# SokhengDin/DNN-MPPI-MPC

Measured on AMD Instinct MI355X. Metric: trajectory-steps/sec (KxT/iter_time), diff-drive K=4096 T=50, higher is better.
Workload: dtype f32; 1 GPU; BASELINE config 2: differential-drive analytic dynamics, K=4096 x T=50 per GPU, reference __main__ parameters, closed loop with the driver's plant on the device; K_per_gpu=4096, K_global=4096, T=50, waypoint_mode=sequential (reference-exact), noise=Philox4x32-10 in-kernel, waypoint_idx_at_end_of_timing=99, build_id=03c7b1dc90acac61, exchange=none (one GPU)

## Files before the change

dnn-mppi-mpc_amd/csrc/mppi_kernels.hip:

```cpp
#include <hip/hip_runtime.h>
#include <limits.h>
#include <math.h>

#include "mppi_device.h"

namespace mppi {

template <typename R> struct alignas(4 * sizeof(R)) VecT4 { R x, y, z, w; };

#ifdef MPPI_STAMPS
__device__ unsigned long long g_stamps[128];
#define STAMP(n)                                                                 \
    do {                                                                         \
        if (blockIdx.x == gridDim.x - 1 && threadIdx.x == 0) g_stamps[64 + (n)] = wall_clock64(); \
        if (blockIdx.x == 0 && threadIdx.x == 0) {                               \
            g_stamps[n] = wall_clock64();                                        \
            if ((n) < 8) g_stamps[40 + (n)] = clock64();  \
            if ((n) == 16 || (n) == 21) g_stamps[32 + (n)] = clock64();           \
        }                                                                        \
    } while (0)
#else
#define STAMP(n) \
    do {         \
    } while (0)
// ... 1342 lines not shown
    }
    eta = wv::reduce<wv::OpAdd>(eta);
    eta2 = wv::reduce<wv::OpAdd>(eta2);
    n_hit = wv::reduce<wv::OpAdd>(n_hit);
    if (lane == 0) { sh_red[4 + wid] = eta; sh_red[8 + wid] = eta2; sh_red[12 + wid] = n_hit; }
    __syncthreads();
    R *out = partials + (size_t)blockIdx.x * record_len(P.T, (int)sizeof(R));
    if (tid == 0) {
        R a = 0, b = 0, nh = 0;
        for (int w = 0; w < nw; ++w) { a += sh_red[4 + w]; b += sh_red[8 + w]; nh += sh_red[12 + w]; }
        out[0] = rho;
        out[1] = a;
        out[2] = b;
        *reinterpret_cast<VecT4<R> *>(P.heads + 4 * (size_t)blockIdx.x) = VecT4<R>{rho, a, b, nh};
    }

    const int n_chunk = (P.T + 63) >> 6;
    for (int ch = 0; ch < n_chunk; ++ch) {
        const int t = ch * 64 + lane;
        R a0 = 0, a1 = 0;
        if (t < P.T) {
            for (int i = wid; i < nk; i += nw) {
                float e0, e1;
                if (P.use_philox) {
                    px::sample(P.seed_lo, P.seed_hi, iter, (unsigned)(k0 + i + P.k_offset), t, P.chol, e0, e1, (unsigned)P.noise_stream);
                } else {
                    const float2 e = *reinterpret_cast<const float2 *>(eps_tensor(P, iter, 0) + ((size_t)(k0 + i) * P.T + t) * 2);
                    e0 = e.x;
                    e1 = e.y;
                }
                const R w = sh_e[i];
                a0 += w * (R)e0;
                a1 += w * (R)e1;
            }
        }
        sh_acc[wid * 128 + 2 * lane] = a0;
        sh_acc[wid * 128 + 2 * lane + 1] = a1;
        __syncthreads();
        if (tid < 128 && ch * 64 + (tid >> 1) < P.T) {
            R s = 0;
            for (int w = 0; w < nw; ++w) s += sh_acc[w * 128 + tid];
            out[4 + ch * 128 + tid] = s;
        }
        __syncthreads();
    }
}

template <typename R>
__global__ void k_weights(const R *__restrict__ S, int K, double beta, double rho, double eta, double *w) {
    const int k = blockIdx.x * blockDim.x + threadIdx.x;
    if (k < K) w[k] = exp(-beta * ((double)S[k] - rho)) / eta;
}

template <int NT> struct MergeShape {
    static constexpr int GROUPS = NT / 32, MAXJ = MERGE_MAX_RECORDS / GROUPS, WAVES = NT / 64;
};

template <typename A> struct alignas(16) VecT { A v[16 / sizeof(A)]; };

template <typename A, int NT = MERGE_THREADS> struct MergeLds {
    A *w, *u, *s, *red, *part;
    __device__ __forceinline__ MergeLds(char *smem, int T, int W) {
        w = reinterpret_cast<A *>(smem);
        u = w + ((2 * (T + W + 1) + 3) & ~3);
        s = u + ((2 * T + 3) & ~3);
        red = s + MERGE_MAX_WINDOWS * NT;
        part = red + 64;
    }
};

__device__ __forceinline__ float fast_exp(float x) { return __expf(x); }
__device__ __forceinline__ double fast_exp(double x) { return exp(x); }
__device__ __forceinline__ float fast_div(float a, float b) { return a * __builtin_amdgcn_rcpf(b); }
__device__ __forceinline__ double fast_div(double a, double b) { return a / b; }

template <typename A> __device__ __forceinline__ void filter_store(A *sh_w, int i, A v, int T, int H, bool pad_copy) {
    const int t = i >> 1, d = i & 1;
    const A pv = pad_copy ? v : A(0);
    sh_w[2 * (t + H) + d] = v;
    if (t < H) sh_w[2 * t + d] = pv;
    if (t >= T - H) sh_w[2 * (t + 2 * H) + d] = pv;
    if (t == T - 1) sh_w[2 * (T + 2 * H) + d] = pv;
}
template <typename A> __device__ __forceinline__ A filter_at(const A *sh_w, int t, int d, int T, int W, int f_filter) {
    const int H = W / 2;
    const A inv_w = fast_div(A(1), (A)W);
    if (f_filter == FILTER_NONE) return sh_w[2 * (t + H) + d];
    if (f_filter == FILTER_TORCH) {
        A sacc = 0;
        for (int q = 0; q < W; ++q) {
            const int m = t - H + q;
            if (m >= 0) sacc += sh_w[2 * m + d] * inv_w;
        }
        return sacc;
    }
    const A *tap = sh_w + 2 * t + d;
    A sacc = 0;
    if (W == 10) {
#pragma unroll
        for (int q = 0; q < 10; ++q) sacc += tap[2 * (9 - q)] * inv_w;
    } else {
        for (int q = 0; q < W; ++q) sacc += tap[2 * (W - 1 - q)] * inv_w;
    }
    if (f_filter == FILTER_DIFF) {
        const int n_conv = (W + 1) / 2;
        if (t == 0) sacc *= fast_div((A)W, (A)n_conv);
        else if (t < n_conv) sacc *= fast_div((A)W, (A)(t + n_conv));
        if (t == T - 1)
            for (int q = 1; q < n_conv; ++q) sacc *= fast_div((A)W, (A)(q + n_conv - (W % 2)));
    }
    return sacc;
}

template <typename A> struct BlockRed {
    static __device__ __forceinline__ A min1(A v, A *sh, int tid) {
        v = wv::reduce<wv::OpMin>(v);
        __syncthreads();
        if ((tid & 63) == 0) sh[tid >> 6] = v;
        __syncthreads();
        A r = sh[0];
#pragma unroll
        for (int w = 1; w < MERGE_THREADS / 64; ++w) r = fmin(r, sh[w]);
        return r;
    }
    static __device__ __forceinline__ void add2(A &a, A &b, A *sh, int tid) {
        a = wv::reduce<wv::OpAdd>(a);
        b = wv::reduce<wv::OpAdd>(b);
        __syncthreads();
        if ((tid & 63) == 0) { sh[tid >> 6] = a; sh[32 + (tid >> 6)] = b; }
        __syncthreads();
        a = 0;
        b = 0;
#pragma unroll
        for (int w = 0; w < MERGE_THREADS / 64; ++w) { a += sh[w]; b += sh[32 + w]; }
    }
};

template <typename A, int NT = MERGE_THREADS, int NWIN = 1> struct MergeRegs {
    VecT<A> w[NWIN][MergeShape<NT>::MAXJ];
    A hr[4 * NWIN], he[4 * NWIN], he2[4 * NWIN];
    A hc[4 * NWIN];
};

template <typename A, int NT, int NWIN>
__device__ __forceinline__ void merge_load_heads(const A *__restrict__ heads, MergeRegs<A, NT, NWIN> &m) {
    const int lane = threadIdx.x & 63;
#pragma unroll
    for (int i = 0; i < 4 * NWIN; ++i) {
        const int b = lane + 64 * i;
        const size_t r = (size_t)b;
        const VecT4<A> hd = *reinterpret_cast<const VecT4<A> *>(heads + 4 * r);
        m.hr[i] = hd.x;
        m.he[i] = hd.y;
        m.he2[i] = hd.z;
        m.hc[i] = hd.w;
    }
}

template <typename A, int NT, int NWIN>
__device__ __forceinline__ void merge_load_tile(const A *__restrict__ recs, int T, int vt, MergeRegs<A, NT, NWIN> &m) {
    constexpr int VW = 16 / sizeof(A), MAXJ = MergeShape<NT>::MAXJ;
    const int tid = threadIdx.x, vc = tid & 31, grp = tid >> 5;
    const unsigned rbytes = (unsigned)record_len(T, (int)sizeof(A)) * (unsigned)sizeof(A);
    const int nvc = (2 * T + VW - 1) / VW;
    const char *base = reinterpret_cast<const char *>(recs);
    const unsigned col = (unsigned)(4 + min(vt * 32 + vc, nvc - 1) * VW) * (unsigned)sizeof(A);
    const unsigned off0 = (unsigned)(grp * MAXJ) * rbytes + col;
#pragma unroll
    for (int win = 0; win < NWIN; ++win)
#pragma unroll
        for (int j = 0; j < MAXJ; ++j)
            m.w[win][j] = *reinterpret_cast<const VecT<A> *>(base + (off0 + (unsigned)(win * MERGE_MAX_RECORDS + j) * rbytes));
}

template <typename A, int NT, int NWIN, typename Store>
__device__ __forceinline__ void merge_combine(const A *__restrict__ recs, int n, int T, A beta,
                                              MergeRegs<A, NT, NWIN> &m, A *sh_s, A *sh_part, A &rho, A &eta, A &eta2,
                                              Store store, A *n_hit = nullptr) {
    constexpr int VW = 16 / sizeof(A), MAXJ = MergeShape<NT>::MAXJ, GROUPS = MergeShape<NT>::GROUPS;
    using V = VecT<A>;
    const int tid = threadIdx.x, lane = tid & 63, wid = tid >> 6;
    const int vc = tid & 31, grp = tid >> 5;
    const int nvc = (2 * T + VW - 1) / VW;
    A lr = A(INFINITY);
#pragma unroll
    for (int i = 0; i < 4 * NWIN; ++i) {
        if (lane + 64 * i >= n) m.hr[i] = A(INFINITY);
        lr = fmin(lr, m.hr[i]);
    }
    rho = wv::reduce<wv::OpMin>(lr);
    STAMP(25);
    A sc[4 * NWIN];
    eta = 0;
    eta2 = 0;
#pragma unroll
    for (int i = 0; i < 4 * NWIN; ++i) {
        sc[i] = lane + 64 * i < n ? fast_exp(-beta * (m.hr[i] - rho)) : A(0);
        eta += sc[i] * m.he[i];
        eta2 += sc[i] * sc[i] * m.he2[i];
    }
    eta = wv::reduce<wv::OpAdd>(eta);
    eta2 = wv::reduce<wv::OpAdd>(eta2);
    if (n_hit && *n_hit >= A(0)) {
        A cnt = 0;
#pragma unroll
        for (int i = 0; i < 4 * NWIN; ++i) cnt += lane + 64 * i < n ? m.hc[i] : A(0);
        *n_hit = wv::reduce<wv::OpAdd>(cnt);
    }
    const int r0 = wid * 2 * MAXJ, slot = r0 >> 6;
    A *my_s = sh_s + wid * 64;
#pragma unroll
    for (int win = 0; win < NWIN; ++win)
        my_s[win * NT + lane] = slot == 0 ? sc[4 * win] : slot == 1 ? sc[4 * win + 1] : slot == 2 ? sc[4 * win + 2] : sc[4 * win + 3];
    __builtin_amdgcn_fence(__ATOMIC_RELEASE, "wavefront");
    __builtin_amdgcn_wave_barrier();
    __builtin_amdgcn_fence(__ATOMIC_ACQUIRE, "wavefront");
    STAMP(26);
    const A *sj_base = my_s + (r0 & 63) + (grp & 1) * MAXJ;
    const A inv_eta = fast_div(A(1), eta);
    const int n_tiles = (nvc + 31) / 32;
    for (int vt = 0; vt < n_tiles; ++vt) {
        V acc;
#pragma unroll
        for (int q = 0; q < VW; ++q) acc.v[q] = 0;
#pragma unroll
        for (int win = 0; win < NWIN; ++win)
#pragma unroll
            for (int j = 0; j < MAXJ; ++j) {
                const A sj = sj_base[win * NT + j];
#pragma unroll
                for (int q = 0; q < VW; ++q) acc.v[q] += sj * m.w[win][j].v[q];
            }
        if (vt > 0) __syncthreads();
        *reinterpret_cast<V *>(sh_part + (grp * 32 + vc) * VW) = acc;
        __syncthreads();
        if (__builtin_expect(vt + 1 < n_tiles, 0)) merge_load_tile<A, NT, NWIN>(recs, T, vt + 1, m);
        for (int e = tid; e < 32 * VW; e += NT) {
            const int i = vt * 32 * VW + e;
            if (i < 2 * T) {
                A t = 0;
#pragma unroll
                for (int g = 0; g < GROUPS; ++g) t += sh_part[g * 32 * VW + e];
                store(i, t * inv_eta);
            }
        }
    }
    __syncthreads();
}

template <typename A, typename Store>
__device__ __forceinline__ void merge_abi(const double *recs, int n, int T, A beta, A *sh_s, A *sh_red, A &rho, A &eta,
                                          A &eta2, Store store, int stride = 0) {
    const int tid = threadIdx.x, plen = stride ? stride : partial_len(T);
    A hr = A(INFINITY), he = 0, he2 = 0;
    if (tid < n) {
        const double *pb = recs + tid * plen;
        hr = (A)pb[0];
        he = (A)pb[1];
        he2 = (A)pb[2];
    }
    rho = BlockRed<A>::min1(hr, sh_red, tid);
    const A sc = tid < n ? fast_exp(-beta * (hr - rho)) : A(0);
    if (tid < n) sh_s[tid] = sc;
    eta = sc * he;
    eta2 = sc * sc * he2;
    BlockRed<A>::add2(eta, eta2, sh_red, tid);
    const A inv_eta = fast_div(A(1), eta);
    for (int i = tid; i < 2 * T; i += MERGE_THREADS) {
        A t = 0;
        for (int b = 0; b < n; ++b) t += sh_s[b] * (A)recs[b * plen + 3 + i];
        store(i, t * inv_eta);
    }
    __syncthreads();
}

template <typename A, bool ABI_OUT>
__global__ __launch_bounds__(MERGE_THREADS) void k_merge(const A *__restrict__ recs, const A *__restrict__ heads, int n,
                                                         int group, int T, A beta, void *__restrict__ out,
                                                         A *__restrict__ out_heads) {
    extern __shared__ __attribute__((aligned(16))) char smem[];
    const MergeLds<A> L(smem, T, 0);
    A *sh_w = L.w;
    const int b0 = blockIdx.x * group, nb = min(group, n - b0);
    const A *mine = recs + (size_t)b0 * record_len(T, (int)sizeof(A));
    MergeRegs<A, MERGE_THREADS, 1> mr;
    merge_load_heads<A, MERGE_THREADS, 1>(heads + 4 * (size_t)b0, mr);
    merge_load_tile<A, MERGE_THREADS, 1>(mine, T, 0, mr);
    A rho, eta, eta2, n_hit = 0;
    merge_combine<A, MERGE_THREADS, 1>(mine, nb, T, beta, mr, L.s, L.part, rho, eta, eta2, [&](int i, A v) { sh_w[i] = v; }, &n_hit);
// ... 12 lines not shown
}

__device__ __forceinline__ char *peer_base(unsigned long long peer_ptr, int p) {
    const unsigned lo = (unsigned)__builtin_amdgcn_readlane((int)(unsigned)peer_ptr, p);
    const unsigned hi = (unsigned)__builtin_amdgcn_readlane((int)(unsigned)(peer_ptr >> 32), p);
    return reinterpret_cast<char *>(((unsigned long long)hi << 32) | lo);
}
__device__ __forceinline__ unsigned long long load_peer_ptrs(const FinalizeParams &F) {
    const int lane = threadIdx.x & 63;
    return lane < F.x_nranks ? reinterpret_cast<unsigned long long>(F.x_peers[lane]) : 0ull;
}

__device__ __forceinline__ bool exchange_flags(const FinalizeParams &F, unsigned long long peer_ptr, size_t slot_off) {
    const int tid = threadIdx.x;
    char *own = peer_base(peer_ptr, F.x_rank);
    __syncthreads();
    if (tid < F.x_nranks) {
        long long *theirs = reinterpret_cast<long long *>(reinterpret_cast<char *>(peer_ptr) + slot_off) + F.x_rank;
        __hip_atomic_store(theirs, F.x_seq, __ATOMIC_RELEASE, __HIP_MEMORY_SCOPE_SYSTEM);
        const long long *mine = reinterpret_cast<const long long *>(own + slot_off) + tid;
        const unsigned long long t0 = wall_clock64();
        while (__hip_atomic_load(mine, __ATOMIC_RELAXED, __HIP_MEMORY_SCOPE_SYSTEM) != F.x_seq) {
            if (wall_clock64() - t0 > (unsigned long long)F.x_timeout) {
                __hip_atomic_store(F.x_err, 1, __ATOMIC_RELAXED, __HIP_MEMORY_SCOPE_AGENT);
                break;
            }
            __builtin_amdgcn_s_sleep(2);
        }
        __builtin_amdgcn_fence(__ATOMIC_ACQUIRE, "");
    }
    __syncthreads();
    return __hip_atomic_load(F.x_err, __ATOMIC_RELAXED, __HIP_MEMORY_SCOPE_AGENT) == 0;
}

__global__ __launch_bounds__(64) void k_exchange_probe(const FinalizeParams F, int *ok_out) {
    const int tid = threadIdx.x, n_chk = 8;
    const size_t slot_off = (size_t)(F.x_seq & 1) * xchg_slot_bytes(F.T, F.x_nranks);
    const size_t recs_off = slot_off + sizeof(long long) * XCHG_MAX_RANKS;
    auto pattern = [&](int rank, int i) { return (double)(F.x_seq * 4096 + rank * 64 + i); };
    const unsigned long long peer_ptr = load_peer_ptrs(F);
    for (int p = 0; p < F.x_nranks; ++p) {
        double *rec = reinterpret_cast<double *>(peer_base(peer_ptr, p) + recs_off) + (size_t)F.x_rank * xchg_rec_len(F.T);
        if (tid < n_chk) rec[tid] = pattern(F.x_rank, tid);
    }
    bool ok = exchange_flags(F, peer_ptr, slot_off);
    const double *recs = reinterpret_cast<const double *>(peer_base(peer_ptr, F.x_rank) + recs_off);
    bool match = true;
    for (int r = 0; r < F.x_nranks; ++r)
        if (tid < n_chk) match &= recs[(size_t)r * xchg_rec_len(F.T) + tid] == pattern(r, tid);
    ok = ok && __ballot(!match) == 0ull;
    if (tid == 0) *ok_out = ok ? 1 : 0;
}

template <typename A, int MODE, int NT, int NWIN, bool PLAIN = false, bool HYPK = false>
__device__ __forceinline__ void finalize_body(const void *partials_pre, const void *heads_pre, const DevState *st_pre,
                                              const void *u_pre, int T_pre, const FinalizeParams &F, char *smem,
                                              int agent) {
    constexpr bool ABI_RECS = MODE == 1, XCHG = MODE == 2;
    const bool f_use_args = !PLAIN && F.use_args, f_sequential = PLAIN || F.sequential, f_plant = PLAIN || F.plant;
    const bool f_raise = !PLAIN && F.raise_at_path_end, f_clamp_u = !PLAIN && F.clamp_u, f_trace = !PLAIN && F.u0_trace != nullptr;
    const int f_model = PLAIN ? (int)MODEL_DIFF : F.model, f_filter = PLAIN ? (int)FILTER_DIFF : F.filter_mode;
    static_assert(MODE == 0 || NT == MERGE_THREADS, "the ABI / exchange variants are 256-thread kernels");
    const int tid = threadIdx.x, lane = tid & 63, wid = tid >> 6;
    const int T = F.T, W = F.filter_window, H = W / 2;
    const MergeLds<A, NT> L(smem, T, W);
    A *sh_w = L.w;
    A *sh_u = L.u;
    DevState *st_out = F.st_out + agent;
    StepResult *res = reinterpret_cast<StepResult *>(reinterpret_cast<char *>(F.res) + (size_t)agent * F.res_stride);
    double *res_u = reinterpret_cast<double *>(res + 1);
    const A *u_in = reinterpret_cast<const A *>(u_pre);
    A *u_out = reinterpret_cast<A *>(F.u_out) + (size_t)agent * 2 * T;
    A *u_hist = reinterpret_cast<A *>(F.u_before) + (size_t)agent * 4 * T;
    const int *pout = F.pout + (size_t)agent * F.K;
    const void *partials = partials_pre;
    const A *ref = reinterpret_cast<const A *>(F.ref);

    STAMP(16);
    static_assert(sizeof(DevState) == 72, "DevState layout");
    const int st_word = reinterpret_cast<const int *>(st_pre)[lane < 18 ? lane : 0];
    const A u_old = tid < 2 * T_pre ? u_in[tid] : A(0);
    unsigned long long peer_ptr = 0;
    if (XCHG) peer_ptr = load_peer_ptrs(F);
    MergeRegs<A, NT, NWIN> mr;
    constexpr int HW = HYP_MAX_BLOCKS / 256;
    uint4 hwords[HW];
#pragma unroll
    for (int i = 0; i < HW; ++i) {
        hwords[i] = uint4{0, 0, 0, 0};
        if (HYPK && 4 * (lane + 64 * i) < F.hyp_blocks) hwords[i] = reinterpret_cast<const uint4 *>(F.hyp_slots)[lane + 64 * i];
    }
    if (!ABI_RECS) {
        merge_load_heads<A, NT, NWIN>(reinterpret_cast<const A *>(heads_pre), mr);
        merge_load_tile<A, NT, NWIN>(reinterpret_cast<const A *>(partials_pre), T_pre, 0, mr);
    }
    STAMP(24);
    DevState sv;
    {
        auto word = [&](int i) { return __builtin_amdgcn_readlane(st_word, i); };
        auto dbl = [&](int i) {
            return __builtin_bit_cast(double, ((long long)word(i + 1) << 32) | (unsigned int)word(i));
        };
        sv.x0[0] = dbl(0); sv.x0[1] = dbl(2); sv.x0[2] = dbl(4); sv.x0[3] = dbl(6);
        sv.p = word(8); sv.c = word(9); sv.k_start = word(10); sv.first_k = word(11);
        sv.round = word(12); sv.path_end = word(13); sv.idx_start = word(14); sv.pad = 0;
        sv.iter = ((long long)word(17) << 32) | (unsigned int)word(16);
    }
    const int fk = sv.first_k, round = sv.round;
    const bool args = f_use_args && round == 0;
    const int c_state = args ? F.c_arg : sv.c;
    const int p_state = (args && !f_sequential) ? F.c_arg : sv.p;
    const int idx_start = args ? F.c_arg : sv.idx_start, path_end = args ? (F.c_arg >= F.n_ref - 1) : sv.path_end;
    const long long iter = sv.iter;
    const double x0v[4] = {args ? F.x0_arg[0] : sv.x0[0], args ? F.x0_arg[1] : sv.x0[1],
                           args ? F.x0_arg[2] : sv.x0[2], args ? F.x0_arg[3] : sv.x0[3]};
    DevState nx = sv;
    nx.x0[0] = x0v[0]; nx.x0[1] = x0v[1]; nx.x0[2] = x0v[2]; nx.x0[3] = x0v[3];
    nx.c = c_state; nx.p = p_state; nx.idx_start = idx_start; nx.path_end = path_end;
    nx.first_k = NO_TRIGGER;
    auto publish = [&]() {
        __syncthreads();
        if (tid == 0 && F.seq) {
            __threadfence_system();
            *reinterpret_cast<volatile long long *>(&res->seq) = F.seq;
        }
    };
    auto leave = [&]() {
        if (tid == 0) *st_out = nx;
        if (u_out != u_in)
            for (int i = tid; i < 2 * T; i += NT) u_out[i] = i == tid ? u_old : u_in[i];
        publish();
    };

    if (XCHG && *reinterpret_cast<volatile int *>(F.x_err)) {
        if (tid == 0) { res->status = STATUS_EXCHANGE_FAILED; res->iter = iter; }
        return leave();
    }
    int c_final = c_state;
    bool hyp_done = false;
    if (HYPK) {
        static_assert(!HYPK || (MODE == 0 && NWIN <= 2 && NT == MERGE_THREADS), "the resolution is part of the plain 256-thread finalize");
        const bool hyp_round = round == 0 && min(F.window, F.n_ref - c_state) > 1;
        if (hyp_round) {
            const unsigned tag = lb_tag(F.lb_seq);
            int mx = 0;
            bool bd = false;
#pragma unroll
            for (int i = 0; i < HW; ++i) {
                const unsigned hw[4] = {hwords[i].x, hwords[i].y, hwords[i].z, hwords[i].w};
#pragma unroll
                for (int j = 0; j < 4; ++j) {
                    if (4 * (lane + 64 * i) + j < F.hyp_blocks) {
                        bd |= (hw[j] & LB_TAG_MASK) != tag || (hw[j] & LB_BAD) != 0u;
                        mx = max(mx, (int)(hw[j] & (LB_BAD - 1)));
                    }
                }
            }
            const int lb_max = wv::reduce<wv::OpMaxInt>(mx);
            const bool lb_bad = __ballot(bd) != 0ull;
            if (lb_bad) {
                nx.k_start = 0;
                nx.c = c_state;
                nx.round = round + 1;
                if (tid == 0) {
                    res->status = STATUS_NEED_ROUND;
                    res->k_next = 0;
                    res->c_next = c_state;
                    res->rounds = round + 1;
                    res->iter = iter;
                }
                return leave();
            }
            c_final = c_state + lb_max;
            hyp_done = true;
        }
    }
    if (!hyp_done && f_sequential && fk != NO_TRIGGER) {
        const int c_new = pout[fk];
        if (fk + 1 < F.K) {
            nx.k_start = fk + 1;
            nx.c = c_new;
            nx.round = round + 1;
            if (tid == 0) {
                res->status = STATUS_NEED_ROUND;
                res->k_next = fk + 1;
                res->c_next = c_new;
                res->rounds = round + 1;
                res->iter = iter;
            }
            return leave();
        }
        c_final = c_new;
    }
    const int p_now = f_sequential ? c_final : p_state;

    A cand_x = 0, cand_y = 0;
    const int wlen_next = min(F.window, F.n_ref - p_now);
    if (wid == 0 && f_plant && lane < wlen_next) {
        cand_x = ref[4 * (p_now + lane)];
        cand_y = ref[4 * (p_now + lane) + 1];
    }
    A sn_yaw = 0, cs_yaw = 1;
    if (f_plant) mf::sincos_((A)x0v[2], sn_yaw, cs_yaw);
    STAMP(17);

    const bool pad_copy = f_filter == FILTER_RACE || f_filter == FILTER_TORCH;
    auto store_w = [&](int i, A v) { filter_store<A>(sh_w, i, v, T, H, pad_copy); };
    A rho, eta, eta2;
    A n_hit = A(-1);
    const bool count_hits = F.count_hits != 0;
    if (ABI_RECS) {
        merge_abi<A>(reinterpret_cast<const double *>(F.partials), F.n_part, T, (A)F.beta, L.s, L.red, rho, eta, eta2,
                     store_w);
    } else if (!XCHG) {
        if (count_hits) n_hit = A(0);
        merge_combine<A, NT, NWIN>(reinterpret_cast<const A *>(partials), F.n_part, T, (A)F.beta, mr, L.s, L.part, rho,
                                   eta, eta2, store_w, &n_hit);
        if (!count_hits) n_hit = A(0);
    } else {
        merge_combine<A, NT, NWIN>(reinterpret_cast<const A *>(partials), F.n_part, T, (A)F.beta, mr, L.s, L.part, rho,
                                   eta, eta2, [&](int i, A v) { sh_u[i] = v; });
        const size_t slot_off = (size_t)(F.x_seq & 1) * xchg_slot_bytes(T, F.x_nranks);
        const size_t rec_off = slot_off + sizeof(long long) * XCHG_MAX_RANKS + sizeof(double) * (size_t)F.x_rank * xchg_rec_len(T);
        for (int p = 0; p < F.x_nranks; ++p) {
            double *rec = reinterpret_cast<double *>(peer_base(peer_ptr, p) + rec_off);
            for (int i = tid; i < 2 * T; i += NT) rec[3 + i] = (double)(sh_u[i] * eta);
            if (tid == 0) { rec[0] = (double)rho; rec[1] = (double)eta; rec[2] = (double)eta2; }
        }
        __builtin_amdgcn_fence(__ATOMIC_RELEASE, "");
        if (!exchange_flags(F, peer_ptr, slot_off)) {
            if (tid == 0) {
                res->status = STATUS_EXCHANGE_FAILED;
                res->rounds = round + 1; res->iter = iter;
            }
            return leave();
        }
        const double *recs = reinterpret_cast<const double *>(peer_base(peer_ptr, F.x_rank) + slot_off + sizeof(long long) * XCHG_MAX_RANKS);
        if (F.x_nranks <= XCHG_LDS_RANKS) {
            double *sh_x = reinterpret_cast<double *>(smem + sizeof(A) * merge_lds_elems(T, W, sizeof(A), NT));
            const int tot = F.x_nranks * xchg_rec_len(T);
            for (int i = tid; i < tot; i += NT) sh_x[i] = recs[i];
            __syncthreads();
            recs = sh_x;
        }
        merge_abi<A>(recs, F.x_nranks, T, (A)F.beta, L.s, L.red, rho, eta, eta2, store_w, xchg_rec_len(T));
    }
    STAMP(18);

    if (f_raise && path_end) {
        nx.k_start = 0;
        nx.round = 0;
        if (tid == 0) {
            res->status = STATUS_PATH_END;
            res->idx_start = idx_start; res->idx_after = p_state; res->path_end = 1;
            res->rounds = round + 1; res->iter = iter;
        }
        return leave();
    }

    for (int i = tid; i < 2 * T; i += NT) {
        const int t = i >> 1, d = i & 1;
        const A f = filter_at<A>(sh_w, t, d, T, W, f_filter);
        const A uo = i == tid ? u_old : u_in[i];
        A un = uo + f;
        if (f_clamp_u) un = mf::clamp(un, d == 0 ? (A)F.umax0 : (A)F.umax1);
        sh_u[i] = un;
    }
    __syncthreads();
    STAMP(19);
    for (int i = tid; i < 2 * T; i += NT) {
        const int t = i >> 1, d = i & 1;
        const A uo = i == tid ? u_old : u_in[i];
        const A shifted = sh_u[2 * (t < T - 1 ? t + 1 : T - 1) + d];
        u_hist[i] = uo;
// ... 17 lines not shown
                xn[0] += v * (double)cs_yaw * F.dt;
                xn[1] += v * (double)sn_yaw * F.dt;
                xn[2] += v / F.wheel_base * (double)mf::tan_(steer) * F.dt;
                xn[3] += (double)accel * F.dt;
            }
        }
        nx.iter = iter + 1;
        nx.k_start = 0;
        nx.round = 0;
        nx.p = p_now;
        if (lane == 0) {
            res->status = STATUS_DONE;
            res->k_next = 0; res->c_next = c_final;
            res->idx_start = idx_start;
            res->idx_after = p_now;
            res->path_end = path_end;
            res->rounds = round + 1;
            res->costs_hyp = hyp_done ? 1 : 0;
            res->n_collided = (int)n_hit;
            res->rho = (double)rho; res->eta = (double)eta; res->ess = (double)(eta * eta / eta2);
            res->u0[0] = (double)u0a; res->u0[1] = (double)u0b;
            for (int q = 0; q < 4; ++q) res->x_next[q] = xn[q];
            if (f_trace && agent == 0) { F.u0_trace[2 * iter] = (double)u0a; F.u0_trace[2 * iter + 1] = (double)u0b; }
            res->iter = iter + 1;
        }
        if (f_plant) {
            double best = INFINITY;
            int bj = INT_MAX;
            if (lane < wlen_next) {
                const double dx = xn[0] - (double)cand_x, dy = xn[1] - (double)cand_y;
                best = dx * dx + dy * dy;
                bj = lane;
            }
            for (int j = lane + 64; j < wlen_next; j += 64) {
                const double dx = xn[0] - (double)ref[4 * (p_now + j)], dy = xn[1] - (double)ref[4 * (p_now + j) + 1];
                const double dd = dx * dx + dy * dy;
                if (dd < best) { best = dd; bj = j; }
            }
            wv::argmin_first(best, bj);
            const int c = p_now + bj;
            nx.x0[0] = xn[0]; nx.x0[1] = xn[1]; nx.x0[2] = xn[2]; nx.x0[3] = xn[3];
            nx.c = c;
            nx.idx_start = c;
            nx.path_end = c >= F.n_ref - 1;
            if (!f_sequential) nx.p = c;
        }
        if (lane == 0) *st_out = nx;
    }
    publish();
    STAMP(21);
}

template <typename A, int MODE, int NWIN, bool MULTI, bool PLAIN = false, bool HYPK = false>
__global__ __launch_bounds__(MERGE_THREADS) void k_finalize(const void *partials_pre, const void *heads_pre,
                                                            const DevState *st_pre, const void *u_pre, int T_pre,
                                                            const FinalizeParams F) {
    extern __shared__ __attribute__((aligned(16))) char smem[];
    if (MULTI) {
        const int a = blockIdx.y;
        const AgentScene sc = F.scenes[a];
        FinalizeParams Fa = F;
        Fa.ref = sc.ref;
        Fa.n_ref = sc.n_ref;
        Fa.count_hits = F.count_hits && sc.n_obs > 0;
        const size_t rec = (size_t)a * F.slots * record_len(T_pre, (int)sizeof(A));
        finalize_body<A, MODE, MERGE_THREADS, NWIN>(reinterpret_cast<const A *>(partials_pre) + rec,
                                                    reinterpret_cast<const A *>(heads_pre) + (size_t)a * F.slots * 4,
                                                    st_pre + a, reinterpret_cast<const A *>(u_pre) + (size_t)a * 2 * T_pre,
                                                    T_pre, Fa, smem, a);
    } else {
        finalize_body<A, MODE, MERGE_THREADS, NWIN, PLAIN, HYPK>(partials_pre, heads_pre, st_pre, u_pre, T_pre, F, smem, 0);
    }
}

__global__ void k_sample(unsigned seed_lo, unsigned seed_hi, unsigned iter, int K, int T, int k_offset, float l00,
                         float l10, float l11, float *__restrict__ eps, unsigned stream_word) {
    const size_t i = (size_t)blockIdx.x * blockDim.x + threadIdx.x;
    if (i >= (size_t)K * T) return;
    const int k = (int)(i / T), t = (int)(i % T);
    const float chol[3] = {l00, l10, l11};
    float e0, e1;
    px::sample(seed_lo, seed_hi, iter, (unsigned)(k + k_offset), t, chol, e0, e1, stream_word);
    reinterpret_cast<float2 *>(eps)[i] = make_float2(e0, e1);
}

template <typename R, int MODEL>
__global__ __launch_bounds__(256) void k_viz(const KParams<R> P, const R *__restrict__ u_before,
                                             const R *__restrict__ u_upd, unsigned iter, float *__restrict__ opt,
                                             float *__restrict__ smp) {
    const int lane = threadIdx.x & 63;
    const int row = blockIdx.x * (blockDim.x >> 6) + (threadIdx.x >> 6) - 1;
    if (row >= P.K) return;
    if (row < 0 && !opt) return;
    if (row >= 0 && !smp) return;
    const DevState *st = P.st;
    constexpr int NX = MODEL == MODEL_RACE ? 4 : 3;
    R cx = (R)st->x0[0], cy = (R)st->x0[1], cyaw = (R)st->x0[2], cvel = MODEL == MODEL_RACE ? (R)st->x0[3] : R(0);
    const bool exploit = (row + P.k_offset) < P.n_exploit;
    float *dst = row < 0 ? opt : smp + (size_t)row * P.T * NX;
    const int n_chunk = (P.T + 63) >> 6;
    for (int ch = 0; ch < n_chunk; ++ch) {
        const int t = ch * 64 + lane;
        const bool act = t < P.T;
        const int tc = (t + P.T - 1) % P.T;
        R v0 = 0, v1 = 0;
        if (act) {
            if (row < 0) {
                v0 = mf::clamp(u_upd[2 * tc], P.umax0);
                v1 = mf::clamp(u_upd[2 * tc + 1], P.umax1);
            } else {
                float e0, e1;
                if (P.use_philox) {
                    px::sample(P.seed_lo, P.seed_hi, iter, (unsigned)(row + P.k_offset), tc, P.chol, e0, e1, (unsigned)P.noise_stream);
                } else {
                    const float2 e = *reinterpret_cast<const float2 *>(eps_tensor(P, iter, 0) + ((size_t)row * P.T + tc) * 2);
                    e0 = e.x;
                    e1 = e.y;
                }
                v0 = exploit ? u_before[2 * tc] + (R)e0 : (R)e0;
                v1 = exploit ? u_before[2 * tc + 1] + (R)e1 : (R)e1;
                v0 = mf::clamp(v0, P.umax0);
                v1 = mf::clamp(v1, P.umax1);
            }
        }
// ... 243 lines not shown
    switch (P.layout & LAYOUT_KIND) {
    case LAYOUT_DUAL:
        p.lookback = !MULTI && MODEL == MODEL_DIFF && P.hyp && !twice;
        p.k = dual_plan<R, MODEL, MULTI, 2>(twice, plain_ok, p.lookback);
        break;
    case LAYOUT_PAIR: p.k = dual_plan<R, MODEL, MULTI, 1>(twice, plain_ok, false); break;
    case LAYOUT_TRI:
        if constexpr (sizeof(R) == 4 && MODEL == MODEL_RACE && !MULTI) {
            const bool share = blocks > 256;
            p.k = plain_ok ? (share ? tri_entry<true, true>() : tri_entry<true, false>())
                           : (share ? tri_entry<false, true>() : tri_entry<false, false>());
        }
        break;
    default:
        {
            const bool plain = P.obstacle_model == OBS_NONE && P.use_philox && P.clamp_rollout && !P.wrap_stage && !P.wrap_term &&
                               !P.per_rollout;
            const int spec = plain ? 2 : P.obstacle_model == OBS_NONE ? 1 : 0;
            p.lookback = !MULTI && MODEL == MODEL_DIFF && P.hyp && P.T <= 64;
            p.k = p.lookback  ? fused_plan<R, MODEL_DIFF, 1, false, true>(spec)
                  : P.T <= 64 ? fused_plan<R, MODEL, 1, MULTI, false>(spec)
                              : fused_plan<R, MODEL, 2, MULTI, false>(spec);
        }
    }
    p.records = blocks;
    p.k.grid = dim3(blocks, MULTI ? P.n_agents : 1);
    return p;
}

template <typename R> RolloutPlan plan_rollout(const KParams<R> &P, bool fused, const Switches &sw) {
    const bool diff = P.model == MODEL_DIFF;
    if (fused) {
        if (P.n_agents > 1) return diff ? plan_fused<R, MODEL_DIFF, true>(P, sw) : plan_fused<R, MODEL_RACE, true>(P, sw);
        return diff ? plan_fused<R, MODEL_DIFF, false>(P, sw) : plan_fused<R, MODEL_RACE, false>(P, sw);
    }
    RolloutPlan p;
    p.k = diff ? rollout_entry<R, MODEL_DIFF>() : rollout_entry<R, MODEL_RACE>();
    p.k.grid = dim3((P.K + 3) / 4);
    p.records = reduce_blocks(P.K, P.traj_per_block);
    return p;
}
template <typename R> void launch_rollout(const RolloutPlan &plan, const KParams<R> &P, void *partials, hipStream_t s) {
    const DevState *st = P.st;
    int n_pass = plan.passes;
    void *args[] = {&st, const_cast<KParams<R> *>(&P), &partials, &n_pass};
    launch_plan(plan.k, args, s);
}

template <typename R> void launch_reduce(const KParams<R> &P, void *partials, int n_blocks, hipStream_t s) {
    const size_t shmem = sizeof(R) * ((size_t)P.traj_per_block + 16 + 4 * 128);
    hipLaunchKernelGGL(k_reduce<R>, dim3(n_blocks), dim3(256), shmem, s, P, (R *)partials);
}

static size_t merge_lds(int T, int W, size_t elem) { return elem * merge_lds_elems(T, W, elem); }

template <typename R, bool ABI_OUT> static KernelLaunch merge_entry() {
    static KernelEntry e("k_merge<%s, %s>", type_name<R>(), KernelEntry::of(ABI_OUT));
    return plan_entry(reinterpret_cast<const void *>(k_merge<R, ABI_OUT>), e, MERGE_THREADS);
}
template <typename R> MergeStep plan_merge(const void *recs, const void *heads, int n, int group, int T, void *out, void *out_heads) {
    MergeStep m;
    m.k = out_heads ? merge_entry<R, false>() : merge_entry<R, true>();
    m.k.grid = dim3((n + group - 1) / group);
    m.k.lds = merge_lds(T, 0, sizeof(R));
    m.recs = recs, m.heads = heads, m.n = n, m.group = group, m.out = out, m.out_heads = out_heads;
    return m;
}
template <typename R> void launch_merge(const MergeStep &m, int T, double beta, hipStream_t s) {
    R b = (R)beta;
    void *args[] = {const_cast<const void **>(&m.recs), const_cast<const void **>(&m.heads), const_cast<int *>(&m.n),
                    const_cast<int *>(&m.group), &T, &b, const_cast<void **>(&m.out), const_cast<void **>(&m.out_heads)};
    launch_plan(m.k, args, s);
}

template <typename R, int MODE, int NWIN, bool MULTI, bool PLAIN = false, bool HYPK = false> static KernelLaunch finalize_entry() {
    static KernelEntry e("k_finalize<%s, %d, %d, %s, %s, %s>", type_name<R>(), MODE, NWIN, KernelEntry::of(MULTI), KernelEntry::of(PLAIN),
                         KernelEntry::of(HYPK));
    return plan_entry(reinterpret_cast<const void *>(k_finalize<R, MODE, NWIN, MULTI, PLAIN, HYPK>), e, MERGE_THREADS);
}
template <typename R> KernelLaunch plan_finalize(const FinalizeParams &F, bool abi_recs, bool lookback) {
    const bool two = merge_tree(F.n_part, true).windows > 1;
    const bool multi = !abi_recs && F.x_nranks <= 1 && F.n_agents > 1;
    const bool plain = F.sequential && F.plant && !F.use_args && !F.raise_at_path_end && !F.clamp_u && F.model == MODEL_DIFF &&
                       !F.u0_trace && F.filter_mode == FILTER_DIFF;
    KernelLaunch k = abi_recs         ? finalize_entry<R, 1, 1, false>()
                     : F.x_nranks > 1 ? (two ? finalize_entry<R, 2, 2, false>() : finalize_entry<R, 2, 1, false>())
                     : multi          ? (two ? finalize_entry<R, 0, 2, true>() : finalize_entry<R, 0, 1, true>())
                     : two            ? (lookback ? finalize_entry<R, 0, 2, false, false, true>() : finalize_entry<R, 0, 2, false>())
                     : lookback       ? (plain ? finalize_entry<R, 0, 1, false, true, true>() : finalize_entry<R, 0, 1, false, false, true>())
                                      : (plain ? finalize_entry<R, 0, 1, false, true, false>() : finalize_entry<R, 0, 1, false>());
    k.grid = dim3(1, multi ? F.n_agents : 1);
    k.lds = merge_lds(F.T, F.filter_window, sizeof(R)) + (F.x_nranks > 1 ? sizeof(double) * XCHG_LDS_RANKS * xchg_rec_len(F.T) : 0) +
            (lookback ? (size_t)HYP_MAX_BLOCKS + 16 : 0);
    return k;
}
void launch_finalize(const KernelLaunch &k, const FinalizeParams &F, hipStream_t s) {
    const DevState *st = F.st;
    void *args[] = {const_cast<const void **>(&F.partials), const_cast<const void **>(&F.heads), &st, const_cast<void **>(&F.u),
                    const_cast<int *>(&F.T), const_cast<FinalizeParams *>(&F)};
    launch_plan(k, args, s);
}

void launch_exchange_probe(const FinalizeParams &F, int *ok_out, hipStream_t s) {
    hipLaunchKernelGGL(k_exchange_probe, dim3(1), dim3(64), 0, s, F, ok_out);
}

template <typename R>
void launch_eval_index(const KParams<R> &P, const R *xy, int stride, int n, int p0, int sequential, int *idx_out, int *p_out,
                       hipStream_t s) {
    hipLaunchKernelGGL(k_eval_index<R>, dim3(sequential ? 1 : (n + 63) / 64), dim3(64), 0, s, P.ref, P.n_ref, P.window, xy,
                       stride, n, p0, sequential, idx_out, p_out);
}
template <typename R>
void launch_eval(const KParams<R> &P, int what, const R *x, const R *v, const int *idx, int n, R *out, hipStream_t s) {
    const dim3 grid((n + 255) / 256), block(256);
    if (P.model == MODEL_DIFF) hipLaunchKernelGGL((k_eval<R, MODEL_DIFF>), grid, block, 0, s, P, what, x, v, idx, n, out);
    else hipLaunchKernelGGL((k_eval<R, MODEL_RACE>), grid, block, 0, s, P, what, x, v, idx, n, out);
}
template <typename R> void launch_eval_filter(const R *xx, R *out, int T, int W, int mode, hipStream_t s) {
    hipLaunchKernelGGL(k_eval_filter<R>, dim3(1), dim3(256), sizeof(R) * 2 * (size_t)(T + W + 2), s, xx, out, T, W, mode);
}
void launch_eval_weights(const double *S, int n, double beta, double *w, hipStream_t s) {
    hipLaunchKernelGGL(k_eval_weights, dim3(1), dim3(256), 0, s, S, n, beta, w);
}
template <typename R> void launch_set_state_dev(const KParams<R> &P, const double *x_dev, int nx, hipStream_t s) {
    hipLaunchKernelGGL(k_set_state_dev<R>, dim3(1), dim3(64), 0, s, P.ref, P.n_ref, P.window, P.sequential, P.st, x_dev, nx);
}

template <typename R> void launch_weights(const KParams<R> &P, double rho, double eta, double *w, hipStream_t s) {
    hipLaunchKernelGGL(k_weights<R>, dim3((P.K + 255) / 256), dim3(256), 0, s, P.S, P.K, (double)P.beta, rho, eta, w);
}

void launch_sample(unsigned seed_lo, unsigned seed_hi, unsigned iter, int K, int T, int k_offset, const float *chol,
                   float *eps_out, hipStream_t s, unsigned stream_word) {
    const size_t n = (size_t)K * T;
    hipLaunchKernelGGL(k_sample, dim3((unsigned)((n + 255) / 256)), dim3(256), 0, s, seed_lo, seed_hi, iter, K, T,
                       k_offset, chol[0], chol[1], chol[2], eps_out, stream_word);
}

template <typename R>
void launch_viz(const KParams<R> &P, const R *u_before, const R *u_upd, long long iter, float *opt, float *smp,
                hipStream_t s) {
    const int rows = P.K + 1, blocks = (rows + 3) / 4;
    if (P.model == MODEL_DIFF)
        hipLaunchKernelGGL((k_viz<R, MODEL_DIFF>), dim3(blocks), dim3(256), 0, s, P, u_before, u_upd, (unsigned)iter,
// ... 31 lines not shown
```

Measured before the change: 22.46 billion trajectory-steps/s.

## Split two-window finalize merge across a doubled workgroup, one window per half

When the finalize kernel merges two record windows, it now launches twice as many threads. Each half of the workgroup loads and holds only one window's record tile in registers, rather than every thread holding both. The first half writes its partial sums to LDS, then the second half adds its window's contribution in place. The aim is to cut per-thread register use and spread the global loads over more waves, at the cost of serialising the two accumulation phases and adding an extra barrier.

```diff
diff --git a/dnn-mppi-mpc_amd/csrc/mppi_kernels.hip b/dnn-mppi-mpc_amd/csrc/mppi_kernels.hip
--- a/dnn-mppi-mpc_amd/csrc/mppi_kernels.hip
+++ b/dnn-mppi-mpc_amd/csrc/mppi_kernels.hip
@@ -1418,9 +1418,11 @@
     if (k < K) w[k] = exp(-beta * ((double)S[k] - rho)) / eta;
 }
 
-template <int NT> struct MergeShape {
-    static constexpr int GROUPS = NT / 32, MAXJ = MERGE_MAX_RECORDS / GROUPS, WAVES = NT / 64;
+template <int NT, bool SPLIT = false> struct MergeShape {
+    static constexpr int GROUPS = (SPLIT ? NT / 2 : NT) / 32, MAXJ = MERGE_MAX_RECORDS / GROUPS, WAVES = NT / 64;
 };
+constexpr bool finalize_split(int mode, int nwin) { return mode == 0 && nwin == 2; }
+constexpr int finalize_threads(int mode, int nwin) { return finalize_split(mode, nwin) ? 2 * MERGE_THREADS : MERGE_THREADS; }
 
 template <typename A> struct alignas(16) VecT { A v[16 / sizeof(A)]; };
 
@@ -1502,14 +1504,14 @@
     }
 };
 
-template <typename A, int NT = MERGE_THREADS, int NWIN = 1> struct MergeRegs {
-    VecT<A> w[NWIN][MergeShape<NT>::MAXJ];
+template <typename A, int NT = MERGE_THREADS, int NWIN = 1, bool SPLIT = false> struct MergeRegs {
+    VecT<A> w[SPLIT ? 1 : NWIN][MergeShape<NT, SPLIT>::MAXJ];
     A hr[4 * NWIN], he[4 * NWIN], he2[4 * NWIN];
     A hc[4 * NWIN];
 };
 
-template <typename A, int NT, int NWIN>
-__device__ __forceinline__ void merge_load_heads(const A *__restrict__ heads, MergeRegs<A, NT, NWIN> &m) {
+template <typename A, int NT, int NWIN, bool SPLIT = false>
+__device__ __forceinline__ void merge_load_heads(const A *__restrict__ heads, MergeRegs<A, NT, NWIN, SPLIT> &m) {
     const int lane = threadIdx.x & 63;
 #pragma unroll
     for (int i = 0; i < 4 * NWIN; ++i) {
@@ -1523,30 +1525,39 @@
     }
 }
 
-template <typename A, int NT, int NWIN>
-__device__ __forceinline__ void merge_load_tile(const A *__restrict__ recs, int T, int vt, MergeRegs<A, NT, NWIN> &m) {
-    constexpr int VW = 16 / sizeof(A), MAXJ = MergeShape<NT>::MAXJ;
-    const int tid = threadIdx.x, vc = tid & 31, grp = tid >> 5;
+template <typename A, int NT, int NWIN, bool SPLIT = false>
+__device__ __forceinline__ void merge_load_tile(const A *__restrict__ recs, int T, int vt, MergeRegs<A, NT, NWIN, SPLIT> &m) {
+    constexpr int VW = 16 / sizeof(A), MAXJ = MergeShape<NT, SPLIT>::MAXJ, GROUPS = MergeShape<NT, SPLIT>::GROUPS;
+    const int tid = threadIdx.x, vc = tid & 31, grp = SPLIT ? (tid >> 5) & (GROUPS - 1) : tid >> 5;
     const unsigned rbytes = (unsigned)record_len(T, (int)sizeof(A)) * (unsigned)sizeof(A);
     const int nvc = (2 * T + VW - 1) / VW;
     const char *base = reinterpret_cast<const char *>(recs);
     const unsigned col = (unsigned)(4 + min(vt * 32 + vc, nvc - 1) * VW) * (unsigned)sizeof(A);
     const unsigned off0 = (unsigned)(grp * MAXJ) * rbytes + col;
-#pragma unroll
-    for (int win = 0; win < NWIN; ++win)
-#pragma unroll
-        for (int j = 0; j < MAXJ; ++j)
-            m.w[win][j] = *reinterpret_cast<const VecT<A> *>(base + (off0 + (unsigned)(win * MERGE_MAX_RECORDS + j) * rbytes));
-}
-
-template <typename A, int NT, int NWIN, typename Store>
+    if constexpr (SPLIT) {
+        const unsigned offw = off0 + (unsigned)((tid >> 8) * MERGE_MAX_RECORDS) * rbytes;
+#pragma unroll
+        for (int j = 0; j < MAXJ; ++j) m.w[0][j] = *reinterpret_cast<const VecT<A> *>(base + (offw + (unsigned)j * rbytes));
+    } else {
+#pragma unroll
+        for (int win = 0; win < NWIN; ++win)
+#pragma unroll
+            for (int j = 0; j < MAXJ; ++j)
+                m.w[win][j] = *reinterpret_cast<const VecT<A> *>(base + (off0 + (unsigned)(win * MERGE_MAX_RECORDS + j) * rbytes));
+    }
+}
+
+template <typename A, int NT, int NWIN, bool SPLIT = false, typename Store>
 __device__ __forceinline__ void merge_combine(const A *__restrict__ recs, int n, int T, A beta,
-                                              MergeRegs<A, NT, NWIN> &m, A *sh_s, A *sh_part, A &rho, A &eta, A &eta2,
+                                              MergeRegs<A, NT, NWIN, SPLIT> &m, A *sh_s, A *sh_part, A &rho, A &eta, A &eta2,
                                               Store store, A *n_hit = nullptr) {
-    constexpr int VW = 16 / sizeof(A), MAXJ = MergeShape<NT>::MAXJ, GROUPS = MergeShape<NT>::GROUPS;
+    constexpr int VW = 16 / sizeof(A), MAXJ = MergeShape<NT, SPLIT>::MAXJ, GROUPS = MergeShape<NT, SPLIT>::GROUPS;
+    static_assert(!SPLIT || (NWIN == 2 && NT == 2 * MERGE_THREADS), "a window per half of the workgroup");
     using V = VecT<A>;
     const int tid = threadIdx.x, lane = tid & 63, wid = tid >> 6;
-    const int vc = tid & 31, grp = tid >> 5;
+    const int vc = tid & 31, grp = SPLIT ? (tid >> 5) & (GROUPS - 1) : tid >> 5;
+    const int my_win = SPLIT ? __builtin_amdgcn_readfirstlane(tid >> 8) : 0;
+    const int wloc = SPLIT ? __builtin_amdgcn_readfirstlane(wid & 3) : wid;
     const int nvc = (2 * T + VW - 1) / VW;
     A lr = A(INFINITY);
 #pragma unroll
@@ -1573,11 +1584,16 @@
         for (int i = 0; i < 4 * NWIN; ++i) cnt += lane + 64 * i < n ? m.hc[i] : A(0);
         *n_hit = wv::reduce<wv::OpAdd>(cnt);
     }
-    const int r0 = wid * 2 * MAXJ, slot = r0 >> 6;
+    const int r0 = wloc * 2 * MAXJ, slot = r0 >> 6;
     A *my_s = sh_s + wid * 64;
-#pragma unroll
-    for (int win = 0; win < NWIN; ++win)
-        my_s[win * NT + lane] = slot == 0 ? sc[4 * win] : slot == 1 ? sc[4 * win + 1] : slot == 2 ? sc[4 * win + 2] : sc[4 * win + 3];
+    if constexpr (SPLIT) {
+        const A s0 = my_win ? sc[4] : sc[0], s1 = my_win ? sc[5] : sc[1], s2 = my_win ? sc[6] : sc[2], s3 = my_win ? sc[7] : sc[3];
+        my_s[lane] = slot == 0 ? s0 : slot == 1 ? s1 : slot == 2 ? s2 : s3;
+    } else {
+#pragma unroll
+        for (int win = 0; win < NWIN; ++win)
+            my_s[win * NT + lane] = slot == 0 ? sc[4 * win] : slot == 1 ? sc[4 * win + 1] : slot == 2 ? sc[4 * win + 2] : sc[4 * win + 3];
+    }
     __builtin_amdgcn_fence(__ATOMIC_RELEASE, "wavefront");
     __builtin_amdgcn_wave_barrier();
     __builtin_amdgcn_fence(__ATOMIC_ACQUIRE, "wavefront");
@@ -1589,18 +1605,39 @@
         V acc;
 #pragma unroll
         for (int q = 0; q < VW; ++q) acc.v[q] = 0;
-#pragma unroll
-        for (int win = 0; win < NWIN; ++win)
-#pragma unroll
-            for (int j = 0; j < MAXJ; ++j) {
-                const A sj = sj_base[win * NT + j];
-#pragma unroll
-                for (int q = 0; q < VW; ++q) acc.v[q] += sj * m.w[win][j].v[q];
-            }
-        if (vt > 0) __syncthreads();
-        *reinterpret_cast<V *>(sh_part + (grp * 32 + vc) * VW) = acc;
+        V *my_part = reinterpret_cast<V *>(sh_part + (grp * 32 + vc) * VW);
+        if constexpr (SPLIT) {
+            auto through_window = [&]() {
+#pragma unroll
+                for (int j = 0; j < MAXJ; ++j) {
+                    const A sj = sj_base[j];
+#pragma unroll
+                    for (int q = 0; q < VW; ++q) acc.v[q] += sj * m.w[0][j].v[q];
+                }
+            };
+            if (my_win == 0) through_window();
+            if (vt > 0) __syncthreads();
+            if (my_win == 0) *my_part = acc;
+            __syncthreads();
+            if (my_win != 0) {
+                acc = *my_part;
+                through_window();
+                *my_part = acc;
+            }
+        } else {
+#pragma unroll
+            for (int win = 0; win < NWIN; ++win)
+#pragma unroll
+                for (int j = 0; j < MAXJ; ++j) {
+                    const A sj = sj_base[win * NT + j];
+#pragma unroll
+                    for (int q = 0; q < VW; ++q) acc.v[q] += sj * m.w[win][j].v[q];
+                }
+            if (vt > 0) __syncthreads();
+            *my_part = acc;
+        }
         __syncthreads();
-        if (__builtin_expect(vt + 1 < n_tiles, 0)) merge_load_tile<A, NT, NWIN>(recs, T, vt + 1, m);
+        if (__builtin_expect(vt + 1 < n_tiles, 0)) merge_load_tile<A, NT, NWIN, SPLIT>(recs, T, vt + 1, m);
         for (int e = tid; e < 32 * VW; e += NT) {
             const int i = vt * 32 * VW + e;
             if (i < 2 * T) {
@@ -1719,7 +1756,7 @@
     if (tid == 0) *ok_out = ok ? 1 : 0;
 }
 
-template <typename A, int MODE, int NT, int NWIN, bool PLAIN = false, bool HYPK = false>
+template <typename A, int MODE, int NT, int NWIN, bool PLAIN = false, bool HYPK = false, bool SPLIT = false>
 __device__ __forceinline__ void finalize_body(const void *partials_pre, const void *heads_pre, const DevState *st_pre,
                                               const void *u_pre, int T_pre, const FinalizeParams &F, char *smem,
                                               int agent) {
@@ -1728,6 +1765,7 @@
     const bool f_raise = !PLAIN && F.raise_at_path_end, f_clamp_u = !PLAIN && F.clamp_u, f_trace = !PLAIN && F.u0_trace != nullptr;
     const int f_model = PLAIN ? (int)MODEL_DIFF : F.model, f_filter = PLAIN ? (int)FILTER_DIFF : F.filter_mode;
     static_assert(MODE == 0 || NT == MERGE_THREADS, "the ABI / exchange variants are 256-thread kernels");
+    static_assert(!SPLIT || MODE == 0, "a window per half of the workgroup: the finalize over the rollout's own records");
     const int tid = threadIdx.x, lane = tid & 63, wid = tid >> 6;
     const int T = F.T, W = F.filter_window, H = W / 2;
     const MergeLds<A, NT> L(smem, T, W);
@@ -1749,7 +1787,7 @@
     const A u_old = tid < 2 * T_pre ? u_in[tid] : A(0);
     unsigned long long peer_ptr = 0;
     if (XCHG) peer_ptr = load_peer_ptrs(F);
-    MergeRegs<A, NT, NWIN> mr;
+    MergeRegs<A, NT, NWIN, SPLIT> mr;
     constexpr int HW = HYP_MAX_BLOCKS / 256;
     uint4 hwords[HW];
 #pragma unroll
@@ -1758,8 +1796,8 @@
         if (HYPK && 4 * (lane + 64 * i) < F.hyp_blocks) hwords[i] = reinterpret_cast<const uint4 *>(F.hyp_slots)[lane + 64 * i];
     }
     if (!ABI_RECS) {
-        merge_load_heads<A, NT, NWIN>(reinterpret_cast<const A *>(heads_pre), mr);
-        merge_load_tile<A, NT, NWIN>(reinterpret_cast<const A *>(partials_pre), T_pre, 0, mr);
+        merge_load_heads<A, NT, NWIN, SPLIT>(reinterpret_cast<const A *>(heads_pre), mr);
+        merge_load_tile<A, NT, NWIN, SPLIT>(reinterpret_cast<const A *>(partials_pre), T_pre, 0, mr);
     }
     STAMP(24);
     DevState sv;
@@ -1806,7 +1844,7 @@
     int c_final = c_state;
     bool hyp_done = false;
     if (HYPK) {
-        static_assert(!HYPK || (MODE == 0 && NWIN <= 2 && NT == MERGE_THREADS), "the resolution is part of the plain 256-thread finalize");
+        static_assert(!HYPK || (MODE == 0 && NWIN <= 2), "the resolution is part of the plain finalize (every wave reduces the words itself)");
         const bool hyp_round = round == 0 && min(F.window, F.n_ref - c_state) > 1;
         if (hyp_round) {
             const unsigned tag = lb_tag(F.lb_seq);
@@ -1881,12 +1919,12 @@
                      store_w);
     } else if (!XCHG) {
         if (count_hits) n_hit = A(0);
-        merge_combine<A, NT, NWIN>(reinterpret_cast<const A *>(partials), F.n_part, T, (A)F.beta, mr, L.s, L.part, rho,
-                                   eta, eta2, store_w, &n_hit);
+        merge_combine<A, NT, NWIN, SPLIT>(reinterpret_cast<const A *>(partials), F.n_part, T, (A)F.beta, mr, L.s, L.part, rho,
+                                          eta, eta2, store_w, &n_hit);
         if (!count_hits) n_hit = A(0);
     } else {
-        merge_combine<A, NT, NWIN>(reinterpret_cast<const A *>(partials), F.n_part, T, (A)F.beta, mr, L.s, L.part, rho,
-                                   eta, eta2, [&](int i, A v) { sh_u[i] = v; });
+        merge_combine<A, NT, NWIN, SPLIT>(reinterpret_cast<const A *>(partials), F.n_part, T, (A)F.beta, mr, L.s, L.part, rho,
+                                          eta, eta2, [&](int i, A v) { sh_u[i] = v; });
         const size_t slot_off = (size_t)(F.x_seq & 1) * xchg_slot_bytes(T, F.x_nranks);
         const size_t rec_off = slot_off + sizeof(long long) * XCHG_MAX_RANKS + sizeof(double) * (size_t)F.x_rank * xchg_rec_len(T);
         for (int p = 0; p < F.x_nranks; ++p) {
@@ -2010,9 +2048,11 @@
 }
 
 template <typename A, int MODE, int NWIN, bool MULTI, bool PLAIN = false, bool HYPK = false>
-__global__ __launch_bounds__(MERGE_THREADS) void k_finalize(const void *partials_pre, const void *heads_pre,
-                                                            const DevState *st_pre, const void *u_pre, int T_pre,
-                                                            const FinalizeParams F) {
+__global__ __launch_bounds__(finalize_threads(MODE, NWIN)) void k_finalize(const void *partials_pre, const void *heads_pre,
+                                                                           const DevState *st_pre, const void *u_pre,
+                                                                           int T_pre, const FinalizeParams F) {
+    constexpr int NT = finalize_threads(MODE, NWIN);
+    constexpr bool SPLIT = finalize_split(MODE, NWIN);
     extern __shared__ __attribute__((aligned(16))) char smem[];
     if (MULTI) {
         const int a = blockIdx.y;
@@ -2022,12 +2062,12 @@
         Fa.n_ref = sc.n_ref;
         Fa.count_hits = F.count_hits && sc.n_obs > 0;
         const size_t rec = (size_t)a * F.slots * record_len(T_pre, (int)sizeof(A));
-        finalize_body<A, MODE, MERGE_THREADS, NWIN>(reinterpret_cast<const A *>(partials_pre) + rec,
-                                                    reinterpret_cast<const A *>(heads_pre) + (size_t)a * F.slots * 4,
-                                                    st_pre + a, reinterpret_cast<const A *>(u_pre) + (size_t)a * 2 * T_pre,
-                                                    T_pre, Fa, smem, a);
+        finalize_body<A, MODE, NT, NWIN, false, false, SPLIT>(reinterpret_cast<const A *>(partials_pre) + rec,
+                                                              reinterpret_cast<const A *>(heads_pre) + (size_t)a * F.slots * 4,
+                                                              st_pre + a, reinterpret_cast<const A *>(u_pre) + (size_t)a * 2 * T_pre,
+                                                              T_pre, Fa, smem, a);
     } else {
-        finalize_body<A, MODE, MERGE_THREADS, NWIN, PLAIN, HYPK>(partials_pre, heads_pre, st_pre, u_pre, T_pre, F, smem, 0);
+        finalize_body<A, MODE, NT, NWIN, PLAIN, HYPK, SPLIT>(partials_pre, heads_pre, st_pre, u_pre, T_pre, F, smem, 0);
     }
 }
 
@@ -2377,7 +2417,7 @@
     hipLaunchKernelGGL(k_reduce<R>, dim3(n_blocks), dim3(256), shmem, s, P, (R *)partials);
 }
 
-static size_t merge_lds(int T, int W, size_t elem) { return elem * merge_lds_elems(T, W, elem); }
+static size_t merge_lds(int T, int W, size_t elem, int nt = MERGE_THREADS) { return elem * merge_lds_elems(T, W, elem, nt); }
 
 template <typename R, bool ABI_OUT> static KernelLaunch merge_entry() {
     static KernelEntry e("k_merge<%s, %s>", type_name<R>(), KernelEntry::of(ABI_OUT));
@@ -2401,7 +2441,7 @@
 template <typename R, int MODE, int NWIN, bool MULTI, bool PLAIN = false, bool HYPK = false> static KernelLaunch finalize_entry() {
     static KernelEntry e("k_finalize<%s, %d, %d, %s, %s, %s>", type_name<R>(), MODE, NWIN, KernelEntry::of(MULTI), KernelEntry::of(PLAIN),
                          KernelEntry::of(HYPK));
-    return plan_entry(reinterpret_cast<const void *>(k_finalize<R, MODE, NWIN, MULTI, PLAIN, HYPK>), e, MERGE_THREADS);
+    return plan_entry(reinterpret_cast<const void *>(k_finalize<R, MODE, NWIN, MULTI, PLAIN, HYPK>), e, finalize_threads(MODE, NWIN));
 }
 template <typename R> KernelLaunch plan_finalize(const FinalizeParams &F, bool abi_recs, bool lookback) {
     const bool two = merge_tree(F.n_part, true).windows > 1;
@@ -2415,7 +2455,7 @@
                      : lookback       ? (plain ? finalize_entry<R, 0, 1, false, true, true>() : finalize_entry<R, 0, 1, false, false, true>())
                                       : (plain ? finalize_entry<R, 0, 1, false, true, false>() : finalize_entry<R, 0, 1, false>());
     k.grid = dim3(1, multi ? F.n_agents : 1);
-    k.lds = merge_lds(F.T, F.filter_window, sizeof(R)) + (F.x_nranks > 1 ? sizeof(double) * XCHG_LDS_RANKS * xchg_rec_len(F.T) : 0) +
+    k.lds = merge_lds(F.T, F.filter_window, sizeof(R), (int)k.block.x) + (F.x_nranks > 1 ? sizeof(double) * XCHG_LDS_RANKS * xchg_rec_len(F.T) : 0) +
             (lookback ? (size_t)HYP_MAX_BLOCKS + 16 : 0);
     return k;
 }
```

Measured after the change: 22.18 billion trajectory-steps/s. 0.988x the previous value.
